# CMU-SAFARI/AirLift

Hardware: AMD Instinct MI355X
Metric: reads/sec remapped (150 bp PE) (higher is better)
Workload: dtype u8/int32 (int8 SW lanes, u64 hashes)

## Files before the change

### airlift_amd/csrc/al_kernels_seed.hip

```cpp
#include <hip/hip_runtime.h>
#include <stdint.h>
#include "al_internal.h"
#include "al_device.h"
#include "al_dev_sort.h"
#include <rocprim/warp/warp_scan.hpp>
typedef rocprim::warp_scan<int32_t, 64> ChainWarpScan;

__device__ __forceinline__ uint64_t d_hash64m(uint64_t key, uint64_t mask)
{
	key = (~key + (key << 21)) & mask; key = key ^ key >> 24;
	key = ((key + (key << 3)) + (key << 8)) & mask; key = key ^ key >> 14;
	key = ((key + (key << 2)) + (key << 4)) & mask; key = key ^ key >> 28;
	key = (key + (key << 31)) & mask;
	return key;
}

template <int W>
__device__ __forceinline__ void
d_sketch(const uint32_t *__restrict__ rd_seq, const uint64_t *__restrict__ rd_off, const uint32_t *__restrict__ rd_len,
         const uint64_t *__restrict__ mini_off, AlAnchor *__restrict__ mini, uint32_t *__restrict__ mini_cnt,
         int n_reads, const int w_arg, int k, int pb)
{
	const int w = W ? W : w_arg;
	extern __shared__ uint64_t lds[];
	const int lane = threadIdx.x;
	const int r = blockIdx.x * 64 + lane;
	uint64_t *ring = lds + lane;
// ... 985 lines not shown
	const uint32_t f = frag_list[blockIdx.x];
	const uint64_t b = big_off[blockIdx.x], n = big_off[blockIdx.x + 1] - b;
	const uint32_t r0 = frag_first[f], r1 = frag_first[f + 1];
	int qlen = 0; for (uint32_t r = r0; r < r1; ++r) qlen += (int)rd_len[r];
	const AlMatch *m = match + mini_off[r0];
	AlAnchor *out = anchors + a_off[f];
	const int sb = rid_bits + pos_bits;
	const uint64_t pmask = (1ULL << pos_bits) - 1, rmask = (1ULL << rid_bits) - 1;
	const uint32_t span = (uint32_t)mini_span;
	int tie = frag_nm[f] > 0x10000u ? 1 : 0;
	for (uint64_t t = threadIdx.x; t < n; t += 256) {
		const uint64_t k = keys[b + t], kx = k >> 16;
		const AlMatch mm = m[(uint32_t)k & 0xffffu];
		AlAnchor a; a.x = (kx >> sb & 1) << 63 | (kx >> pos_bits & rmask) << 32 | (kx & pmask);
		a.y = (a.x >> 63) ? (uint64_t)span << 32 | (uint32_t)(qlen - ((int)(mm.q_pos >> 1) + 1 - (int)span) - 1) : (uint64_t)span << 32 | (mm.q_pos >> 1);
		a.y |= (uint64_t)(mm.flags & 0xff) << AL_SEED_SEG_SHIFT;
		if (mm.flags & (1u << 8)) a.y |= AL_SEED_TANDEM;
		if (t + 1 < n && (keys[b + t + 1] >> 16) == kx) tie = 1;
		out[t] = a;
	}
	if (tie) tie_list[f] = 1u;
}

#define AL_RUN_CAP 8192
#define AL_MERGE_TILE 2048
__device__ __forceinline__ uint32_t d_entry_of(const uint64_t *__restrict__ off, int n, uint64_t b)
{
	uint32_t lo = 0, hi = (uint32_t)n;
	while (hi - lo > 1) { const uint32_t mid = (lo + hi) >> 1; if (off[mid] <= b) lo = mid; else hi = mid; }
	return lo;
}
__global__ void k_big_tiles(const uint32_t *__restrict__ na, int n, uint32_t *__restrict__ nt, unsigned int *__restrict__ max_na, const uint32_t tile)
{
	const int i = blockIdx.x * blockDim.x + threadIdx.x;
	if (i > n) return;
	const uint32_t v = i < n ? na[i] : 0u;
	nt[i] = (v + tile - 1) / tile;
	if (i < n) atomicMax(max_na, v);
}
__global__ void k_big_tile_ent(const uint64_t *__restrict__ tile_off, int n_list, uint32_t n_tile, uint32_t *__restrict__ tile_ent)
{
	const uint32_t b = blockIdx.x * blockDim.x + threadIdx.x;
	if (b < n_tile) tile_ent[b] = d_entry_of(tile_off, n_list, b);
}
template <int PER, int NW, int MCAP>
__global__ void __launch_bounds__(64 * NW)
k_anchor_run_sort(const uint64_t *__restrict__ pos, const uint32_t *__restrict__ frag_first, const uint64_t *__restrict__ mini_off, const AlMatch *__restrict__ match,
                  const uint32_t *__restrict__ frag_nm, const uint32_t *__restrict__ frag_na, const uint32_t *__restrict__ frag_list, int n_list,
// ... 63 lines not shown
#pragma unroll
			for (int j = 0; j < CH; ++j) {
				const uint64_t r = d_match_pos_pick(rr[j], ol[j], fl[j]); const bool rev = (r & 1) != (qb[j] & 1);
				const uint64_t key = ((uint64_t)(rev ? 1 : 0) << sb | (r >> 32) << 32 | (uint32_t)((uint32_t)r >> 1)) << 16 | mi[j];
				k[j0 + j] = LIVE(j0 + j) ? key : UINT64_MAX;
			}
#pragma unroll
			for (int j = 0; j < CH; ++j) asm volatile("" : "+v"(k[j0 + j]));
		}
#undef TT
#undef LIVE
	}
	d_bt_levels<PER, NT, 2>(k, sx, tid);
	__syncthreads();
#pragma unroll
	for (int r = 0; r < PER; ++r) { const int e = tid * PER + r; sx[e + (e >> 4)] = k[r]; }
	__syncthreads();
	uint64_t *out = keys + big_off[ent] + base;
	for (uint32_t t = tid; t < cnt; t += NT) out[t] = sx[t + (t >> 4)];
}
template __global__ void k_anchor_run_sort<16, 8, 1024>(const uint64_t *, const uint32_t *, const uint64_t *, const AlMatch *, const uint32_t *, const uint32_t *, const uint32_t *, int, const uint64_t *, const uint32_t *, const uint64_t *, uint64_t *, uint32_t *, int, uint32_t, uint32_t);

struct RunMergeOut { const uint64_t *a_off, *mini_off; const uint32_t *frag_first, *rd_len; const AlMatch *match; AlAnchor *anchors; uint32_t *tie_list; int rid_bits, mini_span; };
struct RunGeo { uint32_t ent, f, n, o, la, lb, d0, d1; uint64_t A0; int last; bool skip; };
__device__ __forceinline__ RunGeo d_run_geo(const uint32_t blk, const uint32_t *__restrict__ tile_ent, const uint64_t *__restrict__ tile_off, const uint32_t *__restrict__ frag_list,
                                            const uint32_t *__restrict__ frag_na, const uint32_t *__restrict__ frag_nm, const int pass, const uint32_t run_len, const uint32_t tile)
{
	RunGeo g; g.ent = tile_ent[blk]; g.f = frag_list[g.ent]; g.n = frag_na[g.f];
	g.last = 0; while (((uint64_t)run_len << (g.last + 1)) < g.n) ++g.last;
	g.skip = frag_nm[g.f] > 1024u || pass > g.last;
	g.o = (uint32_t)(blk - tile_off[g.ent]) * tile;
	const uint64_t L = (uint64_t)run_len << pass, B0 = (uint64_t)g.o / (2 * L) * (2 * L) + L;
	g.A0 = B0 - L;
	g.la = (uint32_t)(g.n - g.A0 < L ? g.n - g.A0 : L); g.lb = B0 < g.n ? (uint32_t)(g.n - B0 < L ? g.n - B0 : L) : 0u;
	g.d0 = g.o - (uint32_t)g.A0; g.d1 = g.d0 + tile < g.la + g.lb ? g.d0 + tile : g.la + g.lb;
	return g;
}
__global__ void __launch_bounds__(256)
k_anchor_run_cuts(const uint64_t *__restrict__ kin, const uint32_t *__restrict__ frag_list, const uint32_t *__restrict__ tile_ent, uint32_t n_tile, const uint64_t *__restrict__ tile_off,
                  const uint64_t *__restrict__ big_off, const uint32_t *__restrict__ frag_na, const uint32_t *__restrict__ frag_nm, const int pass, const uint32_t run_len, const uint32_t tile, uint32_t *__restrict__ cuts)
{
	const uint32_t blk = blockIdx.x * blockDim.x + threadIdx.x;
	if (blk >= n_tile) return;
	const RunGeo g = d_run_geo(blk, tile_ent, tile_off, frag_list, frag_na, frag_nm, pass, run_len, tile);
	if (g.skip || g.lb == 0) { cuts[blk] = g.d0; return; }
	const uint64_t *A = kin + big_off[g.ent] + g.A0, *B = A + ((uint64_t)run_len << pass);
	const uint32_t d = g.d0;
	uint32_t lo = d > g.lb ? d - g.lb : 0u, hi = d < g.la ? d : g.la;
	while (lo < hi) { const uint32_t mid = (lo + hi) >> 1; if (A[mid] < B[d - 1 - mid]) lo = mid + 1; else hi = mid; }
	cuts[blk] = lo;
}
__global__ void __launch_bounds__(256)
k_anchor_run_merge(const uint64_t *__restrict__ kin, uint64_t *__restrict__ kout, const uint32_t *__restrict__ frag_list, const uint32_t *__restrict__ tile_ent, const uint32_t *__restrict__ cuts, const uint64_t *__restrict__ tile_off,
                   const uint64_t *__restrict__ big_off, const uint32_t *__restrict__ frag_na, const uint32_t *__restrict__ frag_nm, const int pass , const RunMergeOut O, const uint32_t run_len, const uint32_t tile )
{
	constexpr int NT = 256, PER = AL_MERGE_TILE / NT;
	__shared__ uint64_t sk[AL_MERGE_TILE + 1];
	const int tid = threadIdx.x;
	const uint32_t blk = blockIdx.x;
	const RunGeo g = d_run_geo(blk, tile_ent, tile_off, frag_list, frag_na, frag_nm, pass, run_len, tile);
	if (g.skip) return;
	const uint32_t ent = g.ent, f = g.f, n = g.n, o = g.o, la = g.la, lb = g.lb, d0 = g.d0, d1 = g.d1, tot = d1 - d0; const int last = g.last;
	const uint64_t L = (uint64_t)run_len << pass;
	const uint64_t *A = kin + big_off[ent] + g.A0, *B = A + L;
	if (tot == 0) return;
	if (lb == 0 && pass < last) {
		uint64_t *out = kout + big_off[ent] + o;
		for (uint32_t t = tid; t < tot; t += NT) out[t] = A[d0 + t];
		return;
	}
	const uint32_t a0 = lb ? cuts[blk] : d0, a1 = !lb ? d1 : d1 == la + lb ? la : cuts[blk + 1];
	(void)n;
	const uint32_t b0 = d0 - a0, b1 = d1 - a1, na = a1 - a0, nb = b1 - b0;
	{
		uint64_t kk[PER];
#pragma unroll
		for (int r = 0; r < PER; ++r) {
			const uint32_t t = (uint32_t)tid + (uint32_t)r * NT, tc = t < tot ? t : tot - 1u;
			const uint64_t *src = tc < na ? A + a0 + tc : B + b0 + (tc - na);
			kk[r] = *src;
		}
#pragma unroll
		for (int r = 0; r < PER; ++r) asm volatile("" : "+v"(kk[r]));
#pragma unroll
		for (int r = 0; r < PER; ++r) { const uint32_t t = (uint32_t)tid + (uint32_t)r * NT; if (t < tot) sk[t] = kk[r]; }
	}
	__syncthreads();
	uint64_t v[PER];
	{
		const uint64_t *sa = sk, *sb = sk + na;
		const uint32_t d = (uint32_t)tid * PER < tot ? (uint32_t)tid * PER : tot;
		uint32_t lo = d > nb ? d - nb : 0u, hi = d < na ? d : na;
		while (lo < hi) { const uint32_t mid = (lo + hi) >> 1; if (sa[mid] < sb[d - 1 - mid]) lo = mid + 1; else hi = mid; }
		uint32_t ia = lo, ib = d - lo;
		uint64_t ka = ia < na ? sa[ia] : UINT64_MAX, kb = ib < nb ? sb[ib] : UINT64_MAX;
#pragma unroll
		for (int r = 0; r < PER; ++r) {
			const bool ta = ka < kb;
			v[r] = ta ? ka : kb;
			if (ta) { ++ia; ka = ia < na ? sa[ia] : UINT64_MAX; } else { ++ib; kb = ib < nb ? sb[ib] : UINT64_MAX; }
		}
	}
	if (pass < last) {
		uint64_t *out = kout + big_off[ent] + o;
#pragma unroll
		for (int r = 0; r < PER; ++r) { const uint32_t t = (uint32_t)tid * PER + r; if (t < tot) out[t] = v[r]; }
		return;
	}
	uint64_t pred = 0; bool has_pred = false;
	if (tid == 0) { if (a0) { pred = A[a0 - 1]; has_pred = true; } if (b0) { const uint64_t q = B[b0 - 1]; if (!has_pred || q > pred) pred = q; has_pred = true; } }
	__syncthreads();
#pragma unroll
	for (int r = 0; r < PER; ++r) { const uint32_t t = (uint32_t)tid * PER + r; if (t < tot) sk[t + 1] = v[r]; }
	if (tid == 0) sk[0] = has_pred ? pred : ~v[0];
	__syncthreads();
	const uint32_t r0 = O.frag_first[f], r1 = O.frag_first[f + 1];
	int qlen = 0; for (uint32_t r = r0; r < r1; ++r) qlen += (int)O.rd_len[r];
	const AlMatch *m = O.match + O.mini_off[r0];
	AlAnchor *out = O.anchors + O.a_off[f] + o;
	const int sbit = 32 + O.rid_bits; const uint64_t lowmask = (1ULL << sbit) - 1; const uint32_t span = (uint32_t)O.mini_span;
	int tie = 0;
	{
		uint64_t kx[PER]; uint32_t qp[PER], fl[PER];
#pragma unroll
		for (int r = 0; r < PER; ++r) {
			const uint32_t t = (uint32_t)tid + (uint32_t)r * NT, tc = t < tot ? t : tot - 1u;
			const uint64_t key = sk[tc + 1]; kx[r] = key >> 16;
			if (t < tot && (sk[tc] >> 16) == kx[r]) tie = 1;
			const AlMatch mm = m[(uint32_t)key & 0xffffu]; qp[r] = mm.q_pos; fl[r] = mm.flags;
		}
#pragma unroll
		for (int r = 0; r < PER; ++r) asm volatile("" : "+v"(qp[r]), "+v"(fl[r]));
#pragma unroll
		for (int r = 0; r < PER; ++r) {
			const uint32_t t = (uint32_t)tid + (uint32_t)r * NT;
			AlAnchor a; a.x = (kx[r] & lowmask) | (kx[r] >> sbit & 1) << 63;
			a.y = (a.x >> 63) ? (uint64_t)span << 32 | (uint32_t)(qlen - ((int)(qp[r] >> 1) + 1 - (int)span) - 1) : (uint64_t)span << 32 | (qp[r] >> 1);
			a.y |= (uint64_t)(fl[r] & 0xff) << AL_SEED_SEG_SHIFT;
			if (fl[r] & (1u << 8)) a.y |= AL_SEED_TANDEM;
			if (t < tot) out[t] = a;
		}
	}
	if (tie) O.tie_list[f] = 1u;
}

__global__ void __launch_bounds__(64)
k_anchor_sort_small(const uint64_t *__restrict__ pos, const uint32_t *__restrict__ frag_first, const uint32_t *__restrict__ rd_len,
                    const uint64_t *__restrict__ mini_off, const AlMatch *__restrict__ match,
                    const uint32_t *__restrict__ frag_nm, const uint32_t *__restrict__ frag_na, const uint64_t *__restrict__ a_off,
                    AlAnchor *__restrict__ anchors, uint32_t *__restrict__ tie_list, unsigned int *__restrict__ tie_cnt,
                    const uint32_t *__restrict__ frag_list, int n_list, unsigned long long *__restrict__ counters, int mini_span)
{
	const int lane = threadIdx.x;
	if ((int)blockIdx.x >= n_list) return;
	const uint32_t f = frag_list ? frag_list[blockIdx.x] : blockIdx.x;
	const uint32_t n = frag_na[f], n_m = frag_nm[f];
	if (n == 0) return;
	const uint32_t r0 = frag_first[f], r1 = frag_first[f + 1];
	int qlen = 0; for (uint32_t r = r0; r < r1; ++r) qlen += (int)rd_len[r];
	const AlMatch *m = match + mini_off[r0];
	AlAnchor *out = anchors + a_off[f];
	if (n > 64u) { if (lane == 0) tie_list[f] = 1u; return; }
	AlMatch mm; mm.off_lo = 0; mm.n = 0; mm.q_pos = 0; mm.flags = 0;
	if ((uint32_t)lane < n_m) mm = m[lane];
	uint32_t incl = mm.n;
	for (int d = 1; d < 64; d <<= 1) { const uint32_t t = __shfl_up(incl, d); if (lane >= d) incl += t; }
	const uint32_t pre = incl - mm.n;
// ... 1046 lines not shown
```

### airlift_amd/csrc/al_runtime.hip

```cpp
#include <hip/hip_runtime.h>
#include <stdio.h>
#include <stdlib.h>
#include <string.h>
#include <cstring>
#include <algorithm>
#include <functional>
#include <thread>
#include <chrono>
#include "al_internal.h"
#include "al_device.h"
#include <mutex>
#include <vector>
#include "al_runtime.h"
#include "al_prim.h"
#include "al_dev_sort.h"
#include "al_io.h"

extern "C" __global__ void k_sketch(const uint32_t *, const uint64_t *, const uint32_t *, const uint64_t *, AlAnchor *, uint32_t *, int, int, int, int);
extern "C" __global__ void k_seed(const uint64_t *, int, const uint32_t *, const uint32_t *, const uint64_t *, AlAnchor *, const uint32_t *, AlMatch *, uint32_t *, uint32_t *, int32_t *, const uint32_t *, int, int, int, uint32_t *);
#ifndef AL_SPEC_CAP
#define AL_SPEC_CAP 512
#endif
struct SpecOut { AlMatch *match; uint32_t *meta; uint32_t *cnt; uint64_t *cand; uint32_t cap, per, cand_cap; };
struct SpecView { uint32_t *first, *rdlen, *nm, *na, *tie, *list, *n_list; uint64_t *moff, *aoff; };
extern "C" __global__ void k_spec_count(const uint64_t *, int, const uint32_t *, const uint32_t *, const uint64_t *, const AlAnchor *, const uint32_t *, const int32_t *, int, int, uint32_t, SpecOut, int, const uint32_t *);
extern "C" __global__ void k_spec_pick(const uint64_t *, int, const uint32_t *, const uint32_t *, const uint64_t *, const AlAnchor *, const uint32_t *, int, SpecOut);
__global__ void k_spec_layout(const uint32_t *, uint32_t, uint32_t, SpecView);
__global__ void k_spec_mark(const uint32_t *, uint32_t, const uint32_t *, const uint32_t *, uint32_t *, uint32_t *, uint32_t *);
__global__ void k_spec_apply(const uint32_t *, const uint32_t *, const uint64_t *, const AlAnchor *, const uint64_t *, AlAnchor *);
extern "C" __global__ void k_alser_count(const AlAnchor *, const uint64_t *, const uint32_t *, const uint32_t *, const uint32_t *, int, int, unsigned long long *);
extern "C" __global__ void k_rechain_test(const AlAnchor *, const uint64_t *, const uint64_t *, const uint32_t *, const uint32_t *, const int32_t *, const uint32_t *, int, uint32_t *, uint32_t *);
struct TileSched { uint32_t n_items; uint32_t ent[7]; uint32_t item[7]; };
struct CtDefer { uint64_t *off, *uslot; uint32_t *na, *meta, *rel, *fragid, *cls; uint32_t *cnt; uint32_t cap; uint32_t *cmp_list, *cmp_cnt; uint32_t *ctie; };
__global__ void k_frag_meta(const uint32_t *, const uint32_t *, int, uint32_t *);
__global__ void k_chain_tile6(const AlAnchor *, const uint64_t *, const uint32_t *, const uint32_t *, const uint32_t *, const TileSched, const uint32_t *, AlAnchor *, uint64_t *, uint32_t *, uint32_t *, uint32_t *, uint32_t *, const AlParams, const int, unsigned long long *, const int, const CtDefer);
template <int CAP> __global__ void k_chain_coop(const AlAnchor *, AlAnchor *, uint64_t *, uint32_t *, const uint64_t *, const uint32_t *, const uint32_t *, const uint64_t *, const uint32_t *, const uint32_t *, uint32_t *, const uint32_t *, int, const AlParams, unsigned long long *);
__global__ void k_u_compact(const uint32_t *, const uint32_t *, const uint64_t *, uint32_t *, uint64_t *, uint32_t *, const uint32_t *, uint32_t *, uint32_t *);
__global__ void k_uo_fill(const uint32_t *, int, const uint64_t *, const uint32_t *, const uint64_t *, uint32_t *, const uint32_t *);
__global__ void k_fb_meta(const uint32_t *, int, const uint32_t *, const uint32_t *, uint32_t *, uint32_t *);
__global__ void k_fb_reads(const uint32_t *, int, const uint32_t *, const uint32_t *, const uint64_t *, uint32_t *, uint32_t *, uint32_t *);
__global__ void k_fb_copy_in(const uint32_t *, int, const uint64_t *, const uint32_t *, const AlAnchor *, const uint64_t *, AlAnchor *);
__global__ void k_fb_copy_out(const uint32_t *, int, const uint64_t *, const uint64_t *, const uint32_t *, const uint64_t *, const AlAnchor *, uint32_t *, uint64_t *, uint32_t *, AlAnchor *);
template <int CAP> __global__ void k_anchor_sort(const uint64_t *, const uint32_t *, const uint32_t *, const uint64_t *, const AlMatch *, const uint32_t *, const uint32_t *, const uint64_t *, AlAnchor *, uint32_t *, unsigned int *, const uint32_t *, int, unsigned long long *, int);
__global__ void k_anchor_sort_small(const uint64_t *, const uint32_t *, const uint32_t *, const uint64_t *, const AlMatch *, const uint32_t *, const uint32_t *, const uint64_t *, AlAnchor *, uint32_t *, unsigned int *, const uint32_t *, int, unsigned long long *, int);
template <int HCAP, int LANES> __global__ void k_anchor_heap(const uint64_t *, const uint32_t *, const uint32_t *, const uint64_t *, const AlMatch *, const uint32_t *, const uint32_t *, const uint64_t *, AlAnchor *, AlAnchor *, const uint32_t *, const uint32_t *, int, int, unsigned long long *, int, const uint32_t *, uint32_t);
template <int MCAPH, int RING> __global__ void k_anchor_heap_wave(const uint64_t *, const uint32_t *, const uint32_t *, const uint64_t *, const AlMatch *, const uint32_t *, const uint32_t *, const uint64_t *, AlAnchor *, const uint32_t *, const uint32_t *, const uint32_t *, uint32_t, unsigned long long *, int);
template <int NSET, int RING> __global__ void k_anchor_heap_lanes(const uint64_t *, const uint32_t *, const uint32_t *, const uint64_t *, const AlMatch *, const uint32_t *, const uint32_t *, const uint64_t *, AlAnchor *, const uint32_t *, const uint32_t *, const uint32_t *, int, unsigned long long *, int);
template <int CAP> __global__ void k_chain(const AlAnchor *, const uint64_t *, const uint32_t *, const uint32_t *, const uint32_t *, AlAnchor *, uint64_t *, uint32_t *, int32_t *, uint64_t *, const uint32_t *, int, AlParams, unsigned long long *, ChainSeg);
template <int CAPL, int LANES> __global__ void k_chain_lds(const AlAnchor *, const uint64_t *, const uint32_t *, const uint32_t *, const uint32_t *, AlAnchor *, uint64_t *, uint32_t *, uint64_t *, const uint32_t *, int, int, AlParams, unsigned long long *, ChainSeg, uint32_t *, int);
template <int PER, int NW, int MCAP> __global__ void k_anchor_sort_reg(const uint64_t *, const uint32_t *, const uint32_t *, const uint64_t *, const AlMatch *, const uint32_t *, const uint32_t *, const uint64_t *, AlAnchor *, uint32_t *, const uint32_t *, int, int, int);
__global__ void k_anchor_big_expand(const uint64_t *, const uint64_t *, const uint32_t *, const AlMatch *, const uint32_t *, const uint32_t *, int, const uint64_t *, uint64_t *, int, int);
struct RunMergeOut { const uint64_t *a_off, *mini_off; const uint32_t *frag_first, *rd_len; const AlMatch *match; AlAnchor *anchors; uint32_t *tie_list; int rid_bits, mini_span; };
__global__ void k_big_tiles(const uint32_t *, int, uint32_t *, unsigned int *, uint32_t);
template <int PER, int NW, int MCAP> __global__ void k_anchor_run_sort(const uint64_t *, const uint32_t *, const uint64_t *, const AlMatch *, const uint32_t *, const uint32_t *, const uint32_t *, int, const uint64_t *, const uint32_t *, const uint64_t *, uint64_t *, uint32_t *, int, uint32_t, uint32_t);
__global__ void k_big_tile_ent(const uint64_t *, int, uint32_t, uint32_t *);
__global__ void k_anchor_run_cuts(const uint64_t *, const uint32_t *, const uint32_t *, uint32_t, const uint64_t *, const uint64_t *, const uint32_t *, const uint32_t *, int, uint32_t, uint32_t, uint32_t *);
__global__ void k_anchor_run_merge(const uint64_t *, uint64_t *, const uint32_t *, const uint32_t *, const uint32_t *, const uint64_t *, const uint64_t *, const uint32_t *, const uint32_t *, int, RunMergeOut, uint32_t, uint32_t);
__global__ void k_anchor_big_scatter(const uint64_t *, const uint32_t *, int, const uint64_t *, const uint64_t *, const uint64_t *, const uint32_t *, const uint32_t *, const AlMatch *, const uint32_t *, AlAnchor *, uint32_t *, int, int, int);
template <int NW> __global__ void k_seg_scan(const AlAnchor *, const uint64_t *, const uint32_t *, const uint32_t *, const uint32_t *, const uint32_t *, int, AlParams, int, int, const uint64_t *, const uint64_t *, uint32_t *, uint32_t *, uint64_t *, uint32_t *, uint32_t *, const uint32_t *, uint32_t *, uint32_t *, uint32_t *, int, int);
template <int NW> __global__ void k_seg_merge(const uint32_t *, int, const uint64_t *, const uint64_t *, const uint4 *, const uint64_t *, const AlAnchor *, const uint64_t *, uint64_t *, AlAnchor *, uint32_t *, uint32_t *, uint32_t *, const uint32_t *, const uint64_t *, uint64_t *, int, int);
template <int NWV> __global__ void k_chain_order_t(const uint32_t *, int, const uint64_t *, const uint32_t *, uint64_t *, AlAnchor *, const uint64_t *, uint64_t *, AlAnchor *, uint32_t *, uint32_t *, int32_t *, int, int);
__global__ void k_lower_bounds(const uint32_t *, uint32_t, LbThr, uint32_t *);
__global__ void k_collect_flagged(const uint32_t *, int, const uint32_t *, uint32_t *, uint32_t *, const uint32_t *, unsigned long long *);
__global__ void k_collect_flagged_blk(const uint32_t *, int, const uint32_t *, uint32_t *, uint32_t *);

static const char *g_stage_names[ST_N] = { "sketch", "seed_lookup", "scan", "size_order", "anchor_sort_small", "anchor_sort", "anchor_sort_blk", "anchor_sort_big", "anchor_heap",
                                           "chain_lds32", "chain_lds48", "chain_lds64", "chain_lds128", "chain_tile", "chain_deferred", "chain_fallback", "chain_ties", "rechain",
                                           "regs", "ext_prep", "ext_sort", "ext_dp_lane", "ext_dp_g4", "ext_dp_g8", "ext_dp_g12", "ext_dp_g16", "ext_dp_g22", "ext_finish", "map_only", "compact" };
static const char *g_stage_kernels[ST_N] = { "k_sketch", "k_seed", "", "", "k_anchor_sort_small", "", "", "", "",
                                             "", "", "", "", "", "", "", "",  "",
                                             "", "k_ext_prep", "", "", "", "k_ext_dp<8, 256, 128, true>", "k_ext_dp<12, 256, 192, true>", "k_ext_dp<16, 256, 256, true>", "k_ext_dp<22, 256, 352, true>", "k_ext_finish", "", "k_compact" };
extern "C" const char *al_stage_kernel(int i) { return i >= 0 && i < ST_N ? g_stage_kernels[i] : ""; }
extern "C" const char *al_stage_name(int i) { return i >= 0 && i < ST_N ? g_stage_names[i] : ""; }

int al_upload_index(const al_idx_t *mi, int device, AlDevIndex *out)
{
	std::lock_guard<std::mutex> lk(mi->dev_mtx);
	auto it = mi->dev.find(device);
	if (it != mi->dev.end()) { *out = it->second; return 0; }
	AlDevIndex d;
// ... 846 lines not shown
	const uint32_t lb65 = pl.lb65, lb129 = pl.lb129, lb257 = pl.lb257, lb513 = pl.lb513, lb1025 = pl.lb1025, lb2049 = pl.lb2049, lb4097 = pl.lb4097, lb_big = pl.lb_big;
	if (ev(ST_ORDER)) return -1;
	{
		if (c->tie_list.ensure((size_t)c->n_frag + 2)) return -1;
		unsigned int *tie_cnt = nullptr;
		AL_HIP_CHECK(hipMemsetAsync(c->tie_list.p, 0, ((size_t)c->n_frag + 1) * 4, s));
		int rid_bits = 1; while ((1ULL << rid_bits) < c->mi->seq.size()) ++rid_bits;
		hipStream_t sb = c->on(AL_ROLE_OVL0);
		AL_HIP_CHECK(hipEventRecord(c->ev_ovl[0], s)); AL_HIP_CHECK(hipStreamWaitEvent(sb, c->ev_ovl[0], 0));
		int pos_bits = 1; { uint32_t mx = 1; for (const AlSeq &sq : c->mi->seq) mx = std::max(mx, sq.len); while (pos_bits < 31 && (1ULL << pos_bits) < mx) ++pos_bits; }
		const int rank_bits = 64 - 16 - 1 - rid_bits - pos_bits;
		const char *const e3 = al_env().test_big_chunk;
		uint32_t chunk_max = rank_bits >= 31 ? 0x7fffffffu : rank_bits >= 1 ? (1u << rank_bits) : 1u;
		if (e3 && atoi(e3) > 0) chunk_max = std::min<uint32_t>(chunk_max, (uint32_t)atoi(e3));
		uint64_t *const sw = c->seed_who;
		sw[SW_RID_BITS] = (uint64_t)rid_bits; sw[SW_POS_BITS] = (uint64_t)pos_bits; sw[SW_RANK_BITS] = (uint64_t)(rank_bits + 64); sw[SW_NL] = (uint64_t)nl;
		sw[SW_LB65] = lb65; sw[SW_LB129] = lb129; sw[SW_LB257] = lb257; sw[SW_LB513] = lb513; sw[SW_LB1025] = lb1025; sw[SW_LB2049] = lb2049; sw[SW_LB4097] = lb4097; sw[SW_LB_BIG] = lb_big;
		if (rank_bits < 0 && lb_big < (uint32_t)nl) {
			sw[SW_FLAG_ALL] += (uint32_t)nl - lb_big;
			hipLaunchKernelGGL(k_flag_list, dim3(((uint32_t)nl - lb_big + 255) / 256), dim3(256), 0, sb, order + lb_big, (int)((uint32_t)nl - lb_big), c->tie_list.p);
		}
		const int big_merge = al_env().big_merge;
		const bool use_merge = (big_merge == 1 || (big_merge == 2 && !first)) && 33 + rid_bits + 16 <= 64 && lb_big < (uint32_t)nl;
		static uint32_t run_len = 8192, tile = 2048;
		{ static bool once = false; if (!once) { once = true; const char *e = al_env().test_run; unsigned a = 0, b = 0;
		  if (e && sscanf(e, "%u,%u", &a, &b) == 2 && a && b && !(a & (a - 1)) && !(b & (b - 1)) && b <= a && a <= 8192 && b <= 2048) { run_len = a; tile = b; } } }
		if (use_merge) {
			const uint32_t nb = (uint32_t)nl - lb_big;
			unsigned int *const mx_d = (unsigned int *)(c->counters.p + 18);
			if (c->big_na.ensure(nb + 2) || c->big_off.ensure(nb + 2) || c->big_nt.ensure(nb + 2) || c->big_toff.ensure(nb + 2)) return -1;
			AL_HIP_CHECK(hipMemsetAsync(mx_d, 0, 8, sb));
			hipLaunchKernelGGL(k_gather_na, dim3((nb + 256) / 256), dim3(256), 0, sb, c->frag_na.p, order + lb_big, (int)nb, c->big_na.p);
			hipLaunchKernelGGL(k_big_tiles, dim3((nb + 256) / 256), dim3(256), 0, sb, (const uint32_t *)c->big_na.p, (int)nb, c->big_nt.p, mx_d, tile);
			if (scan_u32_to_u64(c, c->big_na.p, c->big_off.p, (int)nb, sb, &c->big_tmp) || scan_u32_to_u64(c, c->big_nt.p, c->big_toff.p, (int)nb, sb, &c->big_tmp)) return -1;
			uint64_t nbig = 0, ntile = 0; unsigned int mx = 0;
			AL_HIP_CHECK(hipMemcpyAsync(&nbig, c->big_off.p + nb, 8, hipMemcpyDeviceToHost, sb));
			AL_HIP_CHECK(hipMemcpyAsync(&ntile, c->big_toff.p + nb, 8, hipMemcpyDeviceToHost, sb));
			AL_HIP_CHECK(hipMemcpyAsync(&mx, mx_d, 4, hipMemcpyDeviceToHost, sb));
			AL_HIP_CHECK(hipStreamSynchronize(sb));
			if (ntile >= (1ULL << 31)) { fprintf(stderr, "[airlift] too many anchors in one batch for the run merge: upload fewer fragments\n"); al_nomem_flag() = true; return -1; }
			if (c->big_k0.ensure((size_t)nbig + 1, false, sb) || c->big_k1.ensure((size_t)nbig + 1, false, sb) || c->big_tent.ensure((size_t)ntile + 1) || c->big_cuts.ensure((size_t)ntile + 2)) return -1;
			const uint32_t nt32 = (uint32_t)ntile;
			hipLaunchKernelGGL(k_big_tile_ent, dim3((nt32 + 255) / 256), dim3(256), 0, sb, (const uint64_t *)c->big_toff.p, (int)nb, nt32, c->big_tent.p);
			hipLaunchKernelGGL(HIP_KERNEL_NAME(k_anchor_run_sort<16, 8, 1024>), dim3(nt32), dim3(512), 0, sb, c->di.pos, c->frag_first.p, c->mini_off.p, c->match.p, c->frag_nm.p, c->frag_na.p,
			                   order + lb_big, (int)nb, (const uint64_t *)c->big_toff.p, (const uint32_t *)c->big_tent.p, (const uint64_t *)c->big_off.p, c->big_k0.p, c->tie_list.p, rid_bits, run_len, tile);
			int n_pass = 1; while (((uint64_t)run_len << n_pass) < mx) ++n_pass;
			sw[SW_MERGE_FRAGS] += nb; sw[SW_MERGE_TILES] += nt32; sw[SW_MERGE_PASSES] += (uint64_t)n_pass;
			const RunMergeOut O{c->a_off.p, c->mini_off.p, c->frag_first.p, c->rd_len.p, c->match.p, c->anchors.p, c->tie_list.p, rid_bits, c->mi->k};
			for (int p = 0; p < n_pass; ++p) {
				const uint64_t *kin = (p & 1) ? c->big_k1.p : c->big_k0.p; uint64_t *kout = (p & 1) ? c->big_k0.p : c->big_k1.p;
				hipLaunchKernelGGL(k_anchor_run_cuts, dim3((nt32 + 255) / 256), dim3(256), 0, sb, kin, order + lb_big, (const uint32_t *)c->big_tent.p, nt32, (const uint64_t *)c->big_toff.p, (const uint64_t *)c->big_off.p,
				                   (const uint32_t *)c->frag_na.p, (const uint32_t *)c->frag_nm.p, p, run_len, tile, c->big_cuts.p);
				hipLaunchKernelGGL(k_anchor_run_merge, dim3(nt32), dim3(256), 0, sb, kin, kout, order + lb_big, (const uint32_t *)c->big_tent.p, (const uint32_t *)c->big_cuts.p, (const uint64_t *)c->big_toff.p,
				                   (const uint64_t *)c->big_off.p, (const uint32_t *)c->frag_na.p, (const uint32_t *)c->frag_nm.p, p, O, run_len, tile);
			}
		}
		for (uint32_t b0 = lb_big; !use_merge && rank_bits >= 0 && b0 < (uint32_t)nl; ) {
			const uint32_t nb = std::min<uint32_t>((uint32_t)nl - b0, chunk_max);
			if (c->big_na.ensure(nb + 2) || c->big_off.ensure(nb + 2)) return -1;
			hipLaunchKernelGGL(k_gather_na, dim3((nb + 256) / 256), dim3(256), 0, sb, c->frag_na.p, order + b0, (int)nb, c->big_na.p);
			if (scan_u32_to_u64(c, c->big_na.p, c->big_off.p, (int)nb, sb, &c->big_tmp)) return -1;
			uint64_t nbig = 0;
			AL_HIP_CHECK(hipMemcpyAsync(&nbig, c->big_off.p + nb, 8, hipMemcpyDeviceToHost, sb));
			AL_HIP_CHECK(hipStreamSynchronize(sb));
			if (c->big_k0.ensure((size_t)nbig + 1, false, sb) || c->big_k1.ensure((size_t)nbig + 1, false, sb)) return -1;
			uint64_t *ka = c->big_k0.p, *kbuf = c->big_k1.p;
			hipLaunchKernelGGL(k_anchor_big_expand, dim3(nb), dim3(256), 0, sb, c->di.pos, c->mini_off.p, c->frag_first.p, c->match.p, c->frag_nm.p,
			                   order + b0, (int)nb, c->big_off.p, ka, rid_bits, pos_bits);
			int rbits = 0; while ((1ULL << rbits) < nb) ++rbits;
			rocprim::double_buffer<uint64_t> dk(ka, kbuf);
			const unsigned end_bit = (unsigned)(16 + 1 + rid_bits + pos_bits + rbits);
			if (al_prim_run(c->big_tmp, [&](void *t, size_t &b) { return rocprim::radix_sort_keys(t, b, dk, (size_t)nbig, 16u, end_bit, sb); })) return -1;
			hipLaunchKernelGGL(k_anchor_big_scatter, dim3(nb), dim3(256), 0, sb, dk.current(), order + b0, (int)nb, c->big_off.p, c->a_off.p,
			                   c->mini_off.p, c->frag_first.p, c->rd_len.p, c->match.p, c->frag_nm.p, c->anchors.p, c->tie_list.p, rid_bits, pos_bits, c->mi->k);
			b0 += nb; sw[SW_RADIX_FRAGS] += nb; ++sw[SW_RADIX_CHUNKS];
		}
		AL_HIP_CHECK(hipEventRecord(c->ev_ovl[1], sb));
// ... 520 lines not shown
```

Before: 16.17 million.

## Use 4-way run merges to halve merge-pass launches for big fragments

Generalizes the pairwise run-merge sort for large anchor fragments to a W-way merge, with W=4 by default. Each tile finds W-way cut points through a joint multi-run binary search, then merges in shared memory through log2(W) pairwise stages. This halves the number of global read/write passes and kernel launches over the key arrays. In exchange, each merge needs more in-tile synchronisation, the cut search is more complex, and the cuts buffer grows by a factor of W.

```diff
diff --git a/airlift_amd/csrc/al_dev_runmerge.h b/airlift_amd/csrc/al_dev_runmerge.h
--- /dev/null
+++ b/airlift_amd/csrc/al_dev_runmerge.h
@@ -0,0 +1,144 @@
+#pragma once
+#include <stdint.h>
+#include "al_dev_deflate.h"
+
+#define AL_RUN_CAP 8192
+#define AL_MERGE_TILE 2048
+#define AL_RUN_WAYS 4
+
+template <int W> AL_DHD int al_rm_launches(uint32_t run_len, uint64_t n)
+{
+	int m = 1;
+	for (uint64_t span = (uint64_t)run_len * W; span < n; span *= W) ++m;
+	return m;
+}
+AL_DHD int al_rm_doublings(uint32_t run_len, uint64_t n) { return al_rm_launches<2>(run_len, n); }
+AL_DHD int al_rm_reads(int launch) { return launch & 1; }
+
+template <int W> struct AlRunGeo {
+	uint32_t n, o;
+	int last;
+	bool done;
+	uint64_t L, G0;
+	uint32_t len[W];
+	int runs;
+	uint32_t tot, d0, d1;
+};
+template <int W> AL_DHD AlRunGeo<W> al_rm_geo(uint32_t n, uint32_t tile_in_frag, int launch, uint32_t run_len, uint32_t tile)
+{
+	AlRunGeo<W> g; g.n = n; g.o = tile_in_frag * tile;
+	g.last = al_rm_launches<W>(run_len, n) - 1;
+	g.done = launch > g.last;
+	g.L = run_len; g.G0 = 0; g.runs = 0; g.tot = g.d0 = g.d1 = 0;
+	for (int i = 0; i < W; ++i) g.len[i] = 0;
+	if (g.done) return g;
+	for (int j = 0; j < launch; ++j) g.L *= W;
+	g.G0 = (uint64_t)g.o / (W * g.L) * (W * g.L);
+	for (int i = 0; i < W; ++i) {
+		const uint64_t s = g.G0 + (uint64_t)i * g.L;
+		g.len[i] = s < n ? (uint32_t)(n - s < g.L ? n - s : g.L) : 0u;
+		g.runs += g.len[i] ? 1 : 0; g.tot += g.len[i];
+	}
+	g.d0 = (uint32_t)(g.o - g.G0); g.d1 = g.tot - g.d0 < tile ? g.tot : g.d0 + tile;
+	return g;
+}
+
+template <int W, class K> AL_DHD void al_rm_cuts(const K &key, const AlRunGeo<W> &g, uint32_t d, uint32_t c[W])
+{
+	uint32_t lo[W], hi[W];
+	for (int i = 0; i < W; ++i) { const uint32_t rest = g.tot - g.len[i]; lo[i] = d > rest ? d - rest : 0u; hi[i] = d < g.len[i] ? d : g.len[i]; }
+	for (;;) {
+		uint32_t m[W]; uint64_t x[W], at[W], open_at = 0; bool open[W], any = false;
+		for (int i = W - 1; i >= 0; --i) { open[i] = lo[i] < hi[i]; m[i] = lo[i] + ((hi[i] - lo[i]) >> 1); at[i] = g.G0 + (uint64_t)i * g.L + m[i]; if (open[i]) { open_at = at[i]; any = true; } }
+		if (!any) break;
+		for (int i = 0; i < W; ++i) x[i] = key(open[i] ? at[i] : open_at);
+		uint32_t nlo[W], nhi[W];
+		for (int j = 0; j < W; ++j) {
+			uint64_t in = 0, out = 0;
+			for (int i = 0; i < W; ++i) {
+				in += open[i] && (i == j || x[i] < x[j]) ? m[i] + 1 : lo[i];
+				out += open[i] && (i == j || x[i] > x[j]) ? m[i] : hi[i];
+			}
+			nhi[j] = open[j] && in > d ? m[j] : hi[j]; nlo[j] = open[j] && out < d ? m[j] + 1 : lo[j];
+		}
+		for (int i = 0; i < W; ++i) { lo[i] = nlo[i]; hi[i] = nhi[i]; }
+	}
+	for (int i = 0; i < W; ++i) c[i] = lo[i];
+}
+
+template <int W, class K> AL_DHD void al_rm_tile_cuts(const K &key, const AlRunGeo<W> &g, uint32_t c[W])
+{
+	for (int i = 0; i < W; ++i) c[i] = 0;
+	c[0] = g.d0;
+	if (!g.done && g.runs > 1 && g.d0 > 0) al_rm_cuts<W>(key, g, g.d0, c);
+}
+template <int W> AL_DHD void al_rm_pieces(const AlRunGeo<W> &g, const uint32_t c0[W], const uint32_t c1[W], uint32_t so[W + 1])
+{
+	so[0] = 0;
+	for (int i = 0; i < W; ++i) so[i + 1] = so[i] + ((g.d1 == g.tot ? g.len[i] : c1[i]) - c0[i]);
+}
+template <int W> AL_DHD uint64_t al_rm_src(const AlRunGeo<W> &g, const uint32_t c0[W], const uint32_t so[W + 1], uint32_t tc)
+{
+	uint64_t idx = g.G0 + c0[0] + tc;
+	for (int i = 1; i < W; ++i) if (tc >= so[i]) idx = g.G0 + (uint64_t)i * g.L + c0[i] + (tc - so[i]);
+	return idx;
+}
+template <int W, class K> AL_DHD uint64_t al_rm_pred(const K &key, const AlRunGeo<W> &g, const uint32_t c0[W], bool &has)
+{
+	uint64_t pred = 0; has = false;
+	for (int i = 0; i < W; ++i) if (c0[i]) { const uint64_t q = key(g.G0 + (uint64_t)i * g.L + c0[i] - 1); if (!has || q > pred) pred = q; has = true; }
+	return pred;
+}
+
+template <int PER> AL_DHD void al_rm_merge_seq(const uint64_t *sa, uint32_t na, const uint64_t *sb, uint32_t nb, uint32_t d, uint32_t skip, uint64_t v[PER])
+{
+	uint32_t lo = d > nb ? d - nb : 0u, hi = d < na ? d : na;
+	while (lo < hi) { const uint32_t mid = (lo + hi) >> 1; if (sa[mid] < sb[d - 1 - mid]) lo = mid + 1; else hi = mid; }
+	uint32_t ia = lo, ib = d - lo;
+	uint64_t ka = ia < na ? sa[ia] : UINT64_MAX, kb = ib < nb ? sb[ib] : UINT64_MAX;
+#pragma unroll
+	for (int r = 0; r < PER; ++r) {
+		const bool ta = ka < kb;
+		v[r] = ta ? ka : kb;
+		if ((uint32_t)r < skip) continue;
+		if (ta) { ++ia; ka = ia < na ? sa[ia] : UINT64_MAX; } else { ++ib; kb = ib < nb ? sb[ib] : UINT64_MAX; }
+	}
+}
+template <int PER> AL_DHD void al_rm_stage(const uint64_t *src, const uint32_t *so, int w, uint32_t tid, uint64_t u[PER])
+{
+	const uint32_t s = tid * PER, e = s + PER;
+#pragma unroll
+	for (int r = 0; r < PER; ++r) u[r] = UINT64_MAX;
+	for (int p = 0; p < w / 2; ++p) {
+		const uint32_t o0 = so[2 * p], o1 = so[2 * p + 1], o2 = so[2 * p + 2];
+		const uint32_t b = s > o0 ? s : o0, t = e < o2 ? e : o2;
+		if (b >= t) continue;
+		uint64_t v[PER];
+		al_rm_merge_seq<PER>(src + o0, o1 - o0, src + o1, o2 - o1, b - o0, b - s, v);
+#pragma unroll
+		for (int r = 0; r < PER; ++r) if (s + r >= b && s + r < t) u[r] = v[r];
+	}
+}
+template <int PER> AL_DHD void al_rm_stage_last(const uint64_t *src, uint32_t mid, uint32_t tot, uint32_t tid, uint64_t v[PER])
+{
+	al_rm_merge_seq<PER>(src, mid, src + mid, tot - mid, tid * PER < tot ? tid * PER : tot, 0u, v);
+}
+
+#if !defined(__HIP_DEVICE_COMPILE__)
+template <int W, int PER> static inline void al_rm_tile_host(uint64_t *buf, uint64_t *tmp, const uint32_t so_in[W + 1], uint32_t nt, uint64_t *out)
+{
+	uint32_t so[W + 1];
+	for (int i = 0; i <= W; ++i) so[i] = so_in[i];
+	const uint32_t tot = so[W];
+	for (int w = W; w > 2; w >>= 1) {
+		for (uint32_t tid = 0; tid < nt; ++tid) al_rm_stage<PER>(buf, so, w, tid, tmp + (size_t)tid * PER);
+		for (uint32_t t = 0; t < tot; ++t) buf[t] = tmp[t];
+		for (int p = 0; p <= w / 2; ++p) so[p] = so[2 * p];
+	}
+	for (uint32_t tid = 0; tid < nt; ++tid) {
+		uint64_t v[PER];
+		al_rm_stage_last<PER>(buf, so[1], tot, tid, v);
+		for (int r = 0; r < PER; ++r) if (tid * PER + r < tot) out[tid * PER + r] = v[r];
+	}
+}
+#endif
diff --git a/airlift_amd/csrc/al_kernels_seed.hip b/airlift_amd/csrc/al_kernels_seed.hip
--- a/airlift_amd/csrc/al_kernels_seed.hip
+++ b/airlift_amd/csrc/al_kernels_seed.hip
@@ -3,6 +3,7 @@
 #include "al_internal.h"
 #include "al_device.h"
 #include "al_dev_sort.h"
+#include "al_dev_runmerge.h"
 #include <rocprim/warp/warp_scan.hpp>
 typedef rocprim::warp_scan<int32_t, 64> ChainWarpScan;
 
@@ -1034,8 +1035,6 @@
 	if (tie) tie_list[f] = 1u;
 }
 
-#define AL_RUN_CAP 8192
-#define AL_MERGE_TILE 2048
 __device__ __forceinline__ uint32_t d_entry_of(const uint64_t *__restrict__ off, int n, uint64_t b)
 {
 	uint32_t lo = 0, hi = (uint32_t)n;
@@ -1145,63 +1144,61 @@
 template __global__ void k_anchor_run_sort<16, 8, 1024>(const uint64_t *, const uint32_t *, const uint64_t *, const AlMatch *, const uint32_t *, const uint32_t *, const uint32_t *, int, const uint64_t *, const uint32_t *, const uint64_t *, uint64_t *, uint32_t *, int, uint32_t, uint32_t);
 
 struct RunMergeOut { const uint64_t *a_off, *mini_off; const uint32_t *frag_first, *rd_len; const AlMatch *match; AlAnchor *anchors; uint32_t *tie_list; int rid_bits, mini_span; };
-struct RunGeo { uint32_t ent, f, n, o, la, lb, d0, d1; uint64_t A0; int last; bool skip; };
-__device__ __forceinline__ RunGeo d_run_geo(const uint32_t blk, const uint32_t *__restrict__ tile_ent, const uint64_t *__restrict__ tile_off, const uint32_t *__restrict__ frag_list,
-                                            const uint32_t *__restrict__ frag_na, const uint32_t *__restrict__ frag_nm, const int pass, const uint32_t run_len, const uint32_t tile)
-{
-	RunGeo g; g.ent = tile_ent[blk]; g.f = frag_list[g.ent]; g.n = frag_na[g.f];
-	g.last = 0; while (((uint64_t)run_len << (g.last + 1)) < g.n) ++g.last;
-	g.skip = frag_nm[g.f] > 1024u || pass > g.last;
-	g.o = (uint32_t)(blk - tile_off[g.ent]) * tile;
-	const uint64_t L = (uint64_t)run_len << pass, B0 = (uint64_t)g.o / (2 * L) * (2 * L) + L;
-	g.A0 = B0 - L;
-	g.la = (uint32_t)(g.n - g.A0 < L ? g.n - g.A0 : L); g.lb = B0 < g.n ? (uint32_t)(g.n - B0 < L ? g.n - B0 : L) : 0u;
-	g.d0 = g.o - (uint32_t)g.A0; g.d1 = g.d0 + tile < g.la + g.lb ? g.d0 + tile : g.la + g.lb;
-	return g;
-}
+template <int W> struct RunGeo { uint32_t ent, f; bool skip; AlRunGeo<W> g; };
+template <int W>
+__device__ __forceinline__ RunGeo<W> d_run_geo(const uint32_t blk, const uint32_t *__restrict__ tile_ent, const uint64_t *__restrict__ tile_off, const uint32_t *__restrict__ frag_list,
+                                               const uint32_t *__restrict__ frag_na, const uint32_t *__restrict__ frag_nm, const int launch, const uint32_t run_len, const uint32_t tile)
+{
+	RunGeo<W> r; r.ent = tile_ent[blk]; r.f = frag_list[r.ent];
+	r.g = al_rm_geo<W>(frag_na[r.f], (uint32_t)(blk - tile_off[r.ent]), launch, run_len, tile);
+	r.skip = frag_nm[r.f] > 1024u || r.g.done;
+	return r;
+}
+template <int W>
 __global__ void __launch_bounds__(256)
 k_anchor_run_cuts(const uint64_t *__restrict__ kin, const uint32_t *__restrict__ frag_list, const uint32_t *__restrict__ tile_ent, uint32_t n_tile, const uint64_t *__restrict__ tile_off,
-                  const uint64_t *__restrict__ big_off, const uint32_t *__restrict__ frag_na, const uint32_t *__restrict__ frag_nm, const int pass, const uint32_t run_len, const uint32_t tile, uint32_t *__restrict__ cuts)
+                  const uint64_t *__restrict__ big_off, const uint32_t *__restrict__ frag_na, const uint32_t *__restrict__ frag_nm, const int launch, const uint32_t run_len, const uint32_t tile, uint32_t *__restrict__ cuts)
 {
 	const uint32_t blk = blockIdx.x * blockDim.x + threadIdx.x;
 	if (blk >= n_tile) return;
-	const RunGeo g = d_run_geo(blk, tile_ent, tile_off, frag_list, frag_na, frag_nm, pass, run_len, tile);
-	if (g.skip || g.lb == 0) { cuts[blk] = g.d0; return; }
-	const uint64_t *A = kin + big_off[g.ent] + g.A0, *B = A + ((uint64_t)run_len << pass);
-	const uint32_t d = g.d0;
-	uint32_t lo = d > g.lb ? d - g.lb : 0u, hi = d < g.la ? d : g.la;
-	while (lo < hi) { const uint32_t mid = (lo + hi) >> 1; if (A[mid] < B[d - 1 - mid]) lo = mid + 1; else hi = mid; }
-	cuts[blk] = lo;
-}
+	const RunGeo<W> R = d_run_geo<W>(blk, tile_ent, tile_off, frag_list, frag_na, frag_nm, launch, run_len, tile);
+	uint32_t c[W];
+	const uint64_t *kf = kin + big_off[R.ent];
+	AlRunGeo<W> g = R.g; if (R.skip) g.done = true;
+	al_rm_tile_cuts<W>([kf](uint64_t i) { return kf[i]; }, g, c);
+#pragma unroll
+	for (int i = 0; i < W; ++i) cuts[(uint64_t)blk * W + i] = c[i];
+}
+template <int W>
 __global__ void __launch_bounds__(256)
 k_anchor_run_merge(const uint64_t *__restrict__ kin, uint64_t *__restrict__ kout, const uint32_t *__restrict__ frag_list, const uint32_t *__restrict__ tile_ent, const uint32_t *__restrict__ cuts, const uint64_t *__restrict__ tile_off,
-                   const uint64_t *__restrict__ big_off, const uint32_t *__restrict__ frag_na, const uint32_t *__restrict__ frag_nm, const int pass , const RunMergeOut O, const uint32_t run_len, const uint32_t tile )
+                   const uint64_t *__restrict__ big_off, const uint32_t *__restrict__ frag_na, const uint32_t *__restrict__ frag_nm, const int launch , const RunMergeOut O, const uint32_t run_len, const uint32_t tile )
 {
 	constexpr int NT = 256, PER = AL_MERGE_TILE / NT;
 	__shared__ uint64_t sk[AL_MERGE_TILE + 1];
 	const int tid = threadIdx.x;
 	const uint32_t blk = blockIdx.x;
-	const RunGeo g = d_run_geo(blk, tile_ent, tile_off, frag_list, frag_na, frag_nm, pass, run_len, tile);
-	if (g.skip) return;
-	const uint32_t ent = g.ent, f = g.f, n = g.n, o = g.o, la = g.la, lb = g.lb, d0 = g.d0, d1 = g.d1, tot = d1 - d0; const int last = g.last;
-	const uint64_t L = (uint64_t)run_len << pass;
-	const uint64_t *A = kin + big_off[ent] + g.A0, *B = A + L;
+	const RunGeo<W> R = d_run_geo<W>(blk, tile_ent, tile_off, frag_list, frag_na, frag_nm, launch, run_len, tile);
+	if (R.skip) return;
+	const AlRunGeo<W> &g = R.g;
+	const uint32_t f = R.f, o = g.o, d0 = g.d0, tot = g.d1 - g.d0; const int last = g.last;
 	if (tot == 0) return;
-	if (lb == 0 && pass < last) {
-		uint64_t *out = kout + big_off[ent] + o;
-		for (uint32_t t = tid; t < tot; t += NT) out[t] = A[d0 + t];
+	const uint64_t *kf = kin + big_off[R.ent];
+	if (g.runs == 1 && launch < last) {
+		uint64_t *out = kout + big_off[R.ent] + o;
+		for (uint32_t t = tid; t < tot; t += NT) out[t] = kf[g.G0 + d0 + t];
 		return;
 	}
-	const uint32_t a0 = lb ? cuts[blk] : d0, a1 = !lb ? d1 : d1 == la + lb ? la : cuts[blk + 1];
-	(void)n;
-	const uint32_t b0 = d0 - a0, b1 = d1 - a1, na = a1 - a0, nb = b1 - b0;
+	uint32_t c0[W], c1[W], so[W + 1];
+#pragma unroll
+	for (int i = 0; i < W; ++i) { c0[i] = cuts[(uint64_t)blk * W + i]; c1[i] = g.d1 == g.tot ? 0u : cuts[(uint64_t)(blk + 1) * W + i]; }
+	al_rm_pieces<W>(g, c0, c1, so);
 	{
 		uint64_t kk[PER];
 #pragma unroll
 		for (int r = 0; r < PER; ++r) {
 			const uint32_t t = (uint32_t)tid + (uint32_t)r * NT, tc = t < tot ? t : tot - 1u;
-			const uint64_t *src = tc < na ? A + a0 + tc : B + b0 + (tc - na);
-			kk[r] = *src;
+			kk[r] = kf[al_rm_src<W>(g, c0, so, tc)];
 		}
 #pragma unroll
 		for (int r = 0; r < PER; ++r) asm volatile("" : "+v"(kk[r]));
@@ -1211,27 +1208,27 @@
 	__syncthreads();
 	uint64_t v[PER];
 	{
-		const uint64_t *sa = sk, *sb = sk + na;
-		const uint32_t d = (uint32_t)tid * PER < tot ? (uint32_t)tid * PER : tot;
-		uint32_t lo = d > nb ? d - nb : 0u, hi = d < na ? d : na;
-		while (lo < hi) { const uint32_t mid = (lo + hi) >> 1; if (sa[mid] < sb[d - 1 - mid]) lo = mid + 1; else hi = mid; }
-		uint32_t ia = lo, ib = d - lo;
-		uint64_t ka = ia < na ? sa[ia] : UINT64_MAX, kb = ib < nb ? sb[ib] : UINT64_MAX;
-#pragma unroll
-		for (int r = 0; r < PER; ++r) {
-			const bool ta = ka < kb;
-			v[r] = ta ? ka : kb;
-			if (ta) { ++ia; ka = ia < na ? sa[ia] : UINT64_MAX; } else { ++ib; kb = ib < nb ? sb[ib] : UINT64_MAX; }
-		}
-	}
-	if (pass < last) {
-		uint64_t *out = kout + big_off[ent] + o;
+#pragma unroll
+		for (int w = W; w > 2; w >>= 1) {
+			uint64_t u[PER];
+			al_rm_stage<PER>(sk, so, w, (uint32_t)tid, u);
+			__syncthreads();
+#pragma unroll
+			for (int r = 0; r < PER; ++r) { const uint32_t t = (uint32_t)tid * PER + r; if (t < tot) sk[t] = u[r]; }
+			__syncthreads();
+#pragma unroll
+			for (int p = 0; p <= w / 2; ++p) so[p] = so[2 * p];
+		}
+		al_rm_stage_last<PER>(sk, so[1], tot, (uint32_t)tid, v);
+	}
+	if (launch < last) {
+		uint64_t *out = kout + big_off[R.ent] + o;
 #pragma unroll
 		for (int r = 0; r < PER; ++r) { const uint32_t t = (uint32_t)tid * PER + r; if (t < tot) out[t] = v[r]; }
 		return;
 	}
 	uint64_t pred = 0; bool has_pred = false;
-	if (tid == 0) { if (a0) { pred = A[a0 - 1]; has_pred = true; } if (b0) { const uint64_t q = B[b0 - 1]; if (!has_pred || q > pred) pred = q; has_pred = true; } }
+	if (tid == 0) pred = al_rm_pred<W>([kf](uint64_t i) { return kf[i]; }, g, c0, has_pred);
 	__syncthreads();
 #pragma unroll
 	for (int r = 0; r < PER; ++r) { const uint32_t t = (uint32_t)tid * PER + r; if (t < tot) sk[t + 1] = v[r]; }
@@ -1266,6 +1263,10 @@
 	}
 	if (tie) O.tie_list[f] = 1u;
 }
+#define INST_RUN_MERGE(W) \
+	template __global__ void k_anchor_run_cuts<W>(const uint64_t *, const uint32_t *, const uint32_t *, uint32_t, const uint64_t *, const uint64_t *, const uint32_t *, const uint32_t *, int, uint32_t, uint32_t, uint32_t *); \
+	template __global__ void k_anchor_run_merge<W>(const uint64_t *, uint64_t *, const uint32_t *, const uint32_t *, const uint32_t *, const uint64_t *, const uint64_t *, const uint32_t *, const uint32_t *, int, RunMergeOut, uint32_t, uint32_t);
+INST_RUN_MERGE(2) INST_RUN_MERGE(AL_RUN_WAYS)
 
 __global__ void __launch_bounds__(64)
 k_anchor_sort_small(const uint64_t *__restrict__ pos, const uint32_t *__restrict__ frag_first, const uint32_t *__restrict__ rd_len,
diff --git a/airlift_amd/csrc/al_runtime.hip b/airlift_amd/csrc/al_runtime.hip
--- a/airlift_amd/csrc/al_runtime.hip
+++ b/airlift_amd/csrc/al_runtime.hip
@@ -14,6 +14,7 @@
 #include "al_runtime.h"
 #include "al_prim.h"
 #include "al_dev_sort.h"
+#include "al_dev_runmerge.h"
 #include "al_io.h"
 
 extern "C" __global__ void k_sketch(const uint32_t *, const uint64_t *, const uint32_t *, const uint64_t *, AlAnchor *, uint32_t *, int, int, int, int);
@@ -54,8 +55,8 @@
 __global__ void k_big_tiles(const uint32_t *, int, uint32_t *, unsigned int *, uint32_t);
 template <int PER, int NW, int MCAP> __global__ void k_anchor_run_sort(const uint64_t *, const uint32_t *, const uint64_t *, const AlMatch *, const uint32_t *, const uint32_t *, const uint32_t *, int, const uint64_t *, const uint32_t *, const uint64_t *, uint64_t *, uint32_t *, int, uint32_t, uint32_t);
 __global__ void k_big_tile_ent(const uint64_t *, int, uint32_t, uint32_t *);
-__global__ void k_anchor_run_cuts(const uint64_t *, const uint32_t *, const uint32_t *, uint32_t, const uint64_t *, const uint64_t *, const uint32_t *, const uint32_t *, int, uint32_t, uint32_t, uint32_t *);
-__global__ void k_anchor_run_merge(const uint64_t *, uint64_t *, const uint32_t *, const uint32_t *, const uint32_t *, const uint64_t *, const uint64_t *, const uint32_t *, const uint32_t *, int, RunMergeOut, uint32_t, uint32_t);
+template <int W> __global__ void k_anchor_run_cuts(const uint64_t *, const uint32_t *, const uint32_t *, uint32_t, const uint64_t *, const uint64_t *, const uint32_t *, const uint32_t *, int, uint32_t, uint32_t, uint32_t *);
+template <int W> __global__ void k_anchor_run_merge(const uint64_t *, uint64_t *, const uint32_t *, const uint32_t *, const uint32_t *, const uint64_t *, const uint64_t *, const uint32_t *, const uint32_t *, int, RunMergeOut, uint32_t, uint32_t);
 __global__ void k_anchor_big_scatter(const uint64_t *, const uint32_t *, int, const uint64_t *, const uint64_t *, const uint64_t *, const uint32_t *, const uint32_t *, const AlMatch *, const uint32_t *, AlAnchor *, uint32_t *, int, int, int);
 template <int NW> __global__ void k_seg_scan(const AlAnchor *, const uint64_t *, const uint32_t *, const uint32_t *, const uint32_t *, const uint32_t *, int, AlParams, int, int, const uint64_t *, const uint64_t *, uint32_t *, uint32_t *, uint64_t *, uint32_t *, uint32_t *, const uint32_t *, uint32_t *, uint32_t *, uint32_t *, int, int);
 template <int NW> __global__ void k_seg_merge(const uint32_t *, int, const uint64_t *, const uint64_t *, const uint4 *, const uint64_t *, const AlAnchor *, const uint64_t *, uint64_t *, AlAnchor *, uint32_t *, uint32_t *, uint32_t *, const uint32_t *, const uint64_t *, uint64_t *, int, int);
@@ -948,9 +949,10 @@
 		}
 		const int big_merge = al_env().big_merge;
 		const bool use_merge = (big_merge == 1 || (big_merge == 2 && !first)) && 33 + rid_bits + 16 <= 64 && lb_big < (uint32_t)nl;
-		static uint32_t run_len = 8192, tile = 2048;
-		{ static bool once = false; if (!once) { once = true; const char *e = al_env().test_run; unsigned a = 0, b = 0;
-		  if (e && sscanf(e, "%u,%u", &a, &b) == 2 && a && b && !(a & (a - 1)) && !(b & (b - 1)) && b <= a && a <= 8192 && b <= 2048) { run_len = a; tile = b; } } }
+		static uint32_t run_len = AL_RUN_CAP, tile = AL_MERGE_TILE; static int ways = AL_RUN_WAYS;
+		{ static bool once = false; if (!once) { once = true; const char *e = al_env().test_run; unsigned a = 0, b = 0, w = 0;
+		  const int nf = e ? sscanf(e, "%u,%u,%u", &a, &b, &w) : 0;
+		  if (nf >= 2 && a && b && !(a & (a - 1)) && !(b & (b - 1)) && b <= a && a <= AL_RUN_CAP && b <= AL_MERGE_TILE) { run_len = a; tile = b; if (nf == 3 && (w == 2 || w == AL_RUN_WAYS)) ways = (int)w; } } }
 		if (use_merge) {
 			const uint32_t nb = (uint32_t)nl - lb_big;
 			unsigned int *const mx_d = (unsigned int *)(c->counters.p + 18);
@@ -965,20 +967,23 @@
 			AL_HIP_CHECK(hipMemcpyAsync(&mx, mx_d, 4, hipMemcpyDeviceToHost, sb));
 			AL_HIP_CHECK(hipStreamSynchronize(sb));
 			if (ntile >= (1ULL << 31)) { fprintf(stderr, "[airlift] too many anchors in one batch for the run merge: upload fewer fragments\n"); al_nomem_flag() = true; return -1; }
-			if (c->big_k0.ensure((size_t)nbig + 1, false, sb) || c->big_k1.ensure((size_t)nbig + 1, false, sb) || c->big_tent.ensure((size_t)ntile + 1) || c->big_cuts.ensure((size_t)ntile + 2)) return -1;
+			if (c->big_k0.ensure((size_t)nbig + 1, false, sb) || c->big_k1.ensure((size_t)nbig + 1, false, sb) || c->big_tent.ensure((size_t)ntile + 1) || c->big_cuts.ensure(((size_t)ntile + 2) * AL_RUN_WAYS)) return -1;
 			const uint32_t nt32 = (uint32_t)ntile;
 			hipLaunchKernelGGL(k_big_tile_ent, dim3((nt32 + 255) / 256), dim3(256), 0, sb, (const uint64_t *)c->big_toff.p, (int)nb, nt32, c->big_tent.p);
 			hipLaunchKernelGGL(HIP_KERNEL_NAME(k_anchor_run_sort<16, 8, 1024>), dim3(nt32), dim3(512), 0, sb, c->di.pos, c->frag_first.p, c->mini_off.p, c->match.p, c->frag_nm.p, c->frag_na.p,
 			                   order + lb_big, (int)nb, (const uint64_t *)c->big_toff.p, (const uint32_t *)c->big_tent.p, (const uint64_t *)c->big_off.p, c->big_k0.p, c->tie_list.p, rid_bits, run_len, tile);
-			int n_pass = 1; while (((uint64_t)run_len << n_pass) < mx) ++n_pass;
-			sw[SW_MERGE_FRAGS] += nb; sw[SW_MERGE_TILES] += nt32; sw[SW_MERGE_PASSES] += (uint64_t)n_pass;
+			const int n_launch = ways == 2 ? al_rm_launches<2>(run_len, mx) : al_rm_launches<AL_RUN_WAYS>(run_len, mx);
+			sw[SW_MERGE_FRAGS] += nb; sw[SW_MERGE_TILES] += nt32; sw[SW_MERGE_PASSES] += (uint64_t)al_rm_doublings(run_len, mx);
 			const RunMergeOut O{c->a_off.p, c->mini_off.p, c->frag_first.p, c->rd_len.p, c->match.p, c->anchors.p, c->tie_list.p, rid_bits, c->mi->k};
-			for (int p = 0; p < n_pass; ++p) {
-				const uint64_t *kin = (p & 1) ? c->big_k1.p : c->big_k0.p; uint64_t *kout = (p & 1) ? c->big_k0.p : c->big_k1.p;
-				hipLaunchKernelGGL(k_anchor_run_cuts, dim3((nt32 + 255) / 256), dim3(256), 0, sb, kin, order + lb_big, (const uint32_t *)c->big_tent.p, nt32, (const uint64_t *)c->big_toff.p, (const uint64_t *)c->big_off.p,
-				                   (const uint32_t *)c->frag_na.p, (const uint32_t *)c->frag_nm.p, p, run_len, tile, c->big_cuts.p);
-				hipLaunchKernelGGL(k_anchor_run_merge, dim3(nt32), dim3(256), 0, sb, kin, kout, order + lb_big, (const uint32_t *)c->big_tent.p, (const uint32_t *)c->big_cuts.p, (const uint64_t *)c->big_toff.p,
-				                   (const uint64_t *)c->big_off.p, (const uint32_t *)c->frag_na.p, (const uint32_t *)c->frag_nm.p, p, O, run_len, tile);
+			for (int p = 0; p < n_launch; ++p) {
+				const uint64_t *kin = al_rm_reads(p) ? c->big_k1.p : c->big_k0.p; uint64_t *kout = al_rm_reads(p) ? c->big_k0.p : c->big_k1.p;
+#define LRUN(W) do { \
+				hipLaunchKernelGGL(HIP_KERNEL_NAME(k_anchor_run_cuts<W>), dim3((nt32 + 255) / 256), dim3(256), 0, sb, kin, order + lb_big, (const uint32_t *)c->big_tent.p, nt32, (const uint64_t *)c->big_toff.p, (const uint64_t *)c->big_off.p, \
+				                   (const uint32_t *)c->frag_na.p, (const uint32_t *)c->frag_nm.p, p, run_len, tile, c->big_cuts.p); \
+				hipLaunchKernelGGL(HIP_KERNEL_NAME(k_anchor_run_merge<W>), dim3(nt32), dim3(256), 0, sb, kin, kout, order + lb_big, (const uint32_t *)c->big_tent.p, (const uint32_t *)c->big_cuts.p, (const uint64_t *)c->big_toff.p, \
+				                   (const uint64_t *)c->big_off.p, (const uint32_t *)c->frag_na.p, (const uint32_t *)c->frag_nm.p, p, O, run_len, tile); } while (0)
+				if (ways == 2) LRUN(2); else LRUN(AL_RUN_WAYS);
+#undef LRUN
 			}
 		}
 		for (uint32_t b0 = lb_big; !use_merge && rank_bits >= 0 && b0 < (uint32_t)nl; ) {
```

Result: no change. 16.32 million, median of 6 (+0.9%).
